# truongp-aws/neuronx-distributed-llama3_2

Measured on AMD Instinct MI355X. Metric: tokens/sec (whole node) Llama-3-8B TP=8 bf16 training at 1/2/4/8 MI355X, higher is better.
Workload: dtype bf16

## Files before the change

### neuronx_distributed_llama3_2_amd/csrc/dense_gemm.hip

```cpp
#include "gemm_tile.h"

#include <cstdlib>
#include <type_traits>

namespace nxd {
namespace dg {

constexpr int BM = 256, BN = 256, BK = 64, NT = 512;
constexpr int REG = 16384;
constexpr int BUF = 4 * REG;
constexpr int LDS_BYTES = 2 * BUF;
constexpr int R_ALO = 0, R_AHI = REG, R_BLO = 2 * REG, R_BHI = 3 * REG;

enum Layout { LNT = 0, LTN = 1 };
enum Epi { BF16 = 0, F32_ACC = 1, F32_ATOMIC = 2 };

struct Params {
  const uint16_t* a;
  const uint16_t* b;
  void* c;
  int M, N, K;
  int64_t lda, ldb, ldc;
  int mt, nt;
  int splits;
  int k_per_split;
  int band;
};

__device__ __forceinline__ int nt_swz(int r) { return (r >> 1) & 7; }

__device__ __forceinline__ bf16x8_t frag_nt(const char* reg, int r0, int s) {
  const int l = threadIdx.x & 63, r = r0 + (l & 15), ch = (l >> 4) + 4 * s;
  return __builtin_bit_cast(bf16x8_t, *reinterpret_cast<const u32x4_t*>(reg + r * 128 + ((ch ^ nt_swz(r)) << 4)));
}
template <int L>
__device__ __forceinline__ bf16x8_t frag(const char* reg, int x0, int s) {
  if constexpr (L == LNT) return frag_nt(reg, x0, s);
  else return frag_tr16<256>(reg, x0, 32 * s);
}

__device__ __forceinline__ void wait_regions(int younger) {
  switch (younger) {
    case 5: asm volatile("s_waitcnt vmcnt(10)" ::: "memory"); break;
    case 4: asm volatile("s_waitcnt vmcnt(8)" ::: "memory"); break;
    case 3: asm volatile("s_waitcnt vmcnt(6)" ::: "memory"); break;
    case 2: asm volatile("s_waitcnt vmcnt(4)" ::: "memory"); break;
    case 1: asm volatile("s_waitcnt vmcnt(2)" ::: "memory"); break;
    default: asm volatile("s_waitcnt vmcnt(0)" ::: "memory"); break;
  }
}

template <int L, int E>
__global__ void __launch_bounds__(NT, 1) gemm_kernel(Params p) {
  __shared__ __attribute__((aligned(16))) char smem[LDS_BYTES];
  const int tiles = p.mt * p.nt;
  const int id = xcd_remap(blockIdx.x, gridDim.x);
  const int split = id / tiles;
  int rt, ct;
  band_raster(id - split * tiles, p.mt, p.nt, p.band, rt, ct);
  const int m0 = rt * BM, n0 = ct * BN;
  const int k_begin = split * p.k_per_split;
  const int k_end = min(p.K, k_begin + p.k_per_split);
  const int nk = (k_end - k_begin) / BK;

  const int wid = threadIdx.x >> 6, lane = threadIdx.x & 63;
  const int wr = wid >> 2, wc = wid & 3;

  f32x4_t acc[4][4][2];
#pragma unroll
  for (int q = 0; q < 4; ++q)
#pragma unroll
    for (int i = 0; i < 4; ++i)
#pragma unroll
      for (int j = 0; j < 2; ++j) acc[q][i][j] = f32x4_t{0.f, 0.f, 0.f, 0.f};

  const uint16_t* sa[2][2];
  const uint16_t* sb[2][2];
#pragma unroll
  for (int h = 0; h < 2; ++h)
#pragma unroll
    for (int j = 0; j < 2; ++j) {
      const int piece = 2 * wid + j;
      if constexpr (L == LNT) {
        const int pr = 8 * piece + (lane >> 3), c = (lane & 7) ^ nt_swz(pr);
        sa[h][j] = p.a + (int64_t)min(m0 + 128 * h + pr, p.M - 1) * p.lda + k_begin + 8 * c;
        sb[h][j] = p.b + (int64_t)min(n0 + 128 * h + pr, p.N - 1) * p.ldb + k_begin + 8 * c;
      } else {
        const int pr = 4 * piece + (lane >> 4), c = (lane & 15) ^ tok_swz(pr);
        sa[h][j] = p.a + (int64_t)(k_begin + pr) * p.lda + min(m0 + 128 * h + 8 * c, p.M - 8);
        sb[h][j] = p.b + (int64_t)(k_begin + pr) * p.ldb + min(n0 + 128 * h + 8 * c, p.N - 8);
      }
    }
  const int64_t adv_a = L == LNT ? (int64_t)BK : (int64_t)BK * p.lda;
  const int64_t adv_b = L == LNT ? (int64_t)BK : (int64_t)BK * p.ldb;
  const uint32_t lds0 = lds_addr(smem);

  auto issue = [&](auto rc, int s) {
    constexpr int R = decltype(rc)::value;
    if (s >= nk) return;
    const uint32_t dst = lds0 + (s & 1) * BUF + (R == 0 ? R_ALO : R == 1 ? R_BLO : R == 2 ? R_BHI : R_AHI) + wid * 2048;
    if constexpr (R == 0 || R == 3) {
      constexpr int h = R == 0 ? 0 : 1;
      const int64_t o = (int64_t)s * adv_a;
      dma16(sa[h][0] + o, __builtin_amdgcn_readfirstlane(dst));
      dma16(sa[h][1] + o, __builtin_amdgcn_readfirstlane(dst + 1024));
    } else {
      constexpr int h = R == 1 ? 0 : 1;
      const int64_t o = (int64_t)s * adv_b;
      dma16(sb[h][0] + o, __builtin_amdgcn_readfirstlane(dst));
      dma16(sb[h][1] + o, __builtin_amdgcn_readfirstlane(dst + 1024));
    }
  };
  const int last = 4 * nk - 1;
  auto wait_for = [&](int need, int max_younger = 4) {
    if (need > last) return;
    wait_regions(min(max_younger, last - need));
  };

  using I0 = std::integral_constant<int, 0>;
  using I1 = std::integral_constant<int, 1>;
  using I2 = std::integral_constant<int, 2>;
  using I3 = std::integral_constant<int, 3>;
  bf16x8_t af[4][2], blo[2][2], bhi[2][2];

  issue(I0{}, 0); issue(I1{}, 0); issue(I2{}, 0); issue(I3{}, 0); issue(I0{}, 1); issue(I1{}, 1); issue(I2{}, 1);
  wait_for(1, 5);
  barrier();
#pragma unroll
  for (int i = 0; i < 4; ++i)
#pragma unroll
    for (int s = 0; s < 2; ++s) af[i][s] = frag<L>(smem + R_ALO, wr * 64 + 16 * i, s);
#pragma unroll
  for (int j = 0; j < 2; ++j)
#pragma unroll
    for (int s = 0; s < 2; ++s) blo[j][s] = frag<L>(smem + R_BLO, wc * 32 + 16 * j, s);
  wait_for(2);
  barrier();
  for (int t = 0; t < nk; ++t) {
    const char* buf = smem + (t & 1) * BUF;
    const char* nbuf = smem + ((t + 1) & 1) * BUF;
    issue(I3{}, t + 1);
#pragma unroll
    for (int s = 0; s < 2; ++s)
#pragma unroll
      for (int i = 0; i < 4; ++i) {
#pragma unroll
        for (int j = 0; j < 2; ++j)
          acc[0][i][j] = __builtin_amdgcn_mfma_f32_16x16x32_bf16(af[i][s], blo[j][s], acc[0][i][j], 0, 0, 0);
        if (i < 2) bhi[i][s] = frag<L>(buf + R_BHI, wc * 32 + 16 * i, s);
      }
    wait_for(4 * t + 3);
    barrier();
    issue(I0{}, t + 2);
#pragma unroll
    for (int s = 0; s < 2; ++s)
#pragma unroll
      for (int i = 0; i < 4; ++i) {
#pragma unroll
        for (int j = 0; j < 2; ++j)
          acc[1][i][j] = __builtin_amdgcn_mfma_f32_16x16x32_bf16(af[i][s], bhi[j][s], acc[1][i][j], 0, 0, 0);
        af[i][s] = frag<L>(buf + R_AHI, wr * 64 + 16 * i, s);
      }
    barrier();
    issue(I1{}, t + 2);
#pragma unroll
    for (int s = 0; s < 2; ++s)
#pragma unroll
      for (int i = 0; i < 4; ++i)
#pragma unroll
        for (int j = 0; j < 2; ++j)
          acc[2][i][j] = __builtin_amdgcn_mfma_f32_16x16x32_bf16(af[i][s], bhi[j][s], acc[2][i][j], 0, 0, 0);
    wait_for(4 * t + 5);
    barrier();
    issue(I2{}, t + 2);
#pragma unroll
    for (int s = 0; s < 2; ++s)
#pragma unroll
      for (int j = 0; j < 2; ++j) {
#pragma unroll
        for (int i = 0; i < 4; ++i) {
          acc[3][i][j] = __builtin_amdgcn_mfma_f32_16x16x32_bf16(af[i][s], blo[j][s], acc[3][i][j], 0, 0, 0);
          if (j == 1) af[i][s] = frag<L>(nbuf + R_ALO, wr * 64 + 16 * i, s);
        }
        blo[j][s] = frag<L>(nbuf + R_BLO, wc * 32 + 16 * j, s);
      }
    wait_for(4 * t + 6);
    barrier();
  }
  asm volatile("s_waitcnt vmcnt(0)" ::: "memory");
  __syncthreads();

  constexpr int LD = 36;
  float* slab = reinterpret_cast<float*>(smem) + wid * (64 * LD);
  const int crow = 4 * (lane >> 4), ccol = lane & 15;
#pragma unroll
  for (int qd = 0; qd < 4; ++qd) {
    const int rh = (qd == 2 || qd == 3) ? 1 : 0, ch = (qd == 1 || qd == 2) ? 1 : 0;
#pragma unroll
    for (int i = 0; i < 4; ++i)
#pragma unroll
      for (int j = 0; j < 2; ++j)
#pragma unroll
        for (int r = 0; r < 4; ++r) slab[(16 * i + crow + r) * LD + 16 * j + ccol] = acc[qd][i][j][r];
    __builtin_amdgcn_wave_barrier();
    const int row0 = m0 + 128 * rh + 64 * wr, col0 = n0 + 128 * ch + 32 * wc;
    if constexpr (E == F32_ATOMIC) {
      const int col = col0 + (lane & 31);
      float* cp = static_cast<float*>(p.c);
#pragma unroll 8
      for (int rr = 0; rr < 32; ++rr) {
        const int lr = 2 * rr + (lane >> 5), row = row0 + lr;
        const float v = slab[lr * LD + (lane & 31)];
        if (row < p.M && col < p.N) unsafeAtomicAdd(cp + (int64_t)row * p.ldc + col, v);
      }
    } else {
#pragma unroll
      for (int ps = 0; ps < 4; ++ps) {
        const int lr = 16 * ps + (lane >> 2), c8 = 8 * (lane & 3);
        const int row = row0 + lr, col = col0 + c8;
        const f32x4_t v0 = *reinterpret_cast<const f32x4_t*>(slab + lr * LD + c8);
        const f32x4_t v1 = *reinterpret_cast<const f32x4_t*>(slab + lr * LD + c8 + 4);
        if (row < p.M && col < p.N) {
          if constexpr (E == BF16) {
            u32x4_t o;
            o[0] = pack2bf(v0[0], v0[1]); o[1] = pack2bf(v0[2], v0[3]);
            o[2] = pack2bf(v1[0], v1[1]); o[3] = pack2bf(v1[2], v1[3]);
            *reinterpret_cast<u32x4_t*>(static_cast<uint16_t*>(p.c) + (int64_t)row * p.ldc + col) = o;
          } else {
            f32x4_t* cp = reinterpret_cast<f32x4_t*>(static_cast<float*>(p.c) + (int64_t)row * p.ldc + col);
            const f32x4_t c0 = cp[0], c1 = cp[1];
            cp[0] = c0 + v0;
            cp[1] = c1 + v1;
          }
        }
      }
    }
    __builtin_amdgcn_wave_barrier();
  }
}

static int env_int(const char* name, int dflt) {
  const char* e = getenv(name);
  return e ? atoi(e) : dflt;
}

}

int dense_gemm_choose_splits(int M, int N, int K) {
  const int tiles = ceil_div(M, dg::BM) * ceil_div(N, dg::BN);
  const int steps = K / dg::BK;
  const int64_t base = (int64_t)ceil_div(tiles, 256) * steps;
  int best = 1;
  int64_t best_cost = base;
  for (int s = 2; s <= 8 && s <= steps; ++s) {
    if (steps / s < 8) break;
    const int64_t cost = (int64_t)ceil_div(tiles * s, 256) * (ceil_div(steps, s) + 6);
    if (cost * 10 < best_cost * 9 && cost < best_cost) {
      best_cost = cost;
      best = s;
    }
  }
  return best;
}

int dense_gemm_launch(int layout, int epi, const void* a, int64_t lda, const void* b, int64_t ldb, void* c, int64_t ldc,
                      int M, int N, int K, int splits, hipStream_t stream) {
  if (M <= 0 || N <= 0 || K <= 0) return 0;
  if (K % dg::BK || N % 8 || lda % 8 || ldb % 8 || ldc % 4) return -1;
  if (layout == dg::LTN && M % 8) return -1;
  if (epi == dg::BF16 && ldc % 8) return -1;
  dg::Params p{};
  p.a = static_cast<const uint16_t*>(a);
  p.b = static_cast<const uint16_t*>(b);
  p.c = c;
  p.M = M; p.N = N; p.K = K;
  p.lda = lda; p.ldb = ldb; p.ldc = ldc;
  p.mt = ceil_div(M, dg::BM);
  p.nt = ceil_div(N, dg::BN);
  const int steps = K / dg::BK;
  if (epi != dg::F32_ATOMIC) splits = 1;
  else if (splits <= 0) splits = dense_gemm_choose_splits(M, N, K);
  splits = splits < 1 ? 1 : (splits > steps ? steps : splits);
  p.k_per_split = ceil_div(steps, splits) * dg::BK;
  p.splits = ceil_div(K, p.k_per_split);
  static const int band = [] { const int v = dg::env_int("NXD_DG_BAND", 8); return v > 0 ? v : 8; }();
  p.band = band;
  const int64_t nwg = (int64_t)p.mt * p.nt * p.splits;
  if (nwg > INT32_MAX) return -2;
#define NXD_DG_LAUNCH(LY, EP) \
  hipLaunchKernelGGL((dg::gemm_kernel<LY, EP>), dim3((unsigned)nwg), dim3(dg::NT), 0, stream, p)
  if (layout == dg::LNT) {
    if (epi == dg::BF16) NXD_DG_LAUNCH(dg::LNT, dg::BF16);
    else if (epi == dg::F32_ACC) NXD_DG_LAUNCH(dg::LNT, dg::F32_ACC);
    else NXD_DG_LAUNCH(dg::LNT, dg::F32_ATOMIC);
  } else {
    if (epi == dg::BF16) NXD_DG_LAUNCH(dg::LTN, dg::BF16);
    else if (epi == dg::F32_ACC) NXD_DG_LAUNCH(dg::LTN, dg::F32_ACC);
    else NXD_DG_LAUNCH(dg::LTN, dg::F32_ATOMIC);
  }
#undef NXD_DG_LAUNCH
  return hipGetLastError() == hipSuccess ? 0 : -3;
}

}
```

### neuronx_distributed_llama3_2_amd/ops/gemm.py

```python

from __future__ import annotations

import os

import torch

from ._ext import ext, use_native

_ENABLED = os.environ.get("NXD_TUNED_GEMM", "1") == "1"


def set_overlap_safe(enabled: bool) -> None:
    if not torch.cuda.is_available():
        return
    try:
        ext().gemm_set_no_streamk(1 if enabled else 0)
    except Exception:
        pass


def _native(*t: torch.Tensor) -> bool:
    return _ENABLED and use_native(*t) and all(x.dtype in (torch.bfloat16, torch.float16) for x in t)


def linear(x: torch.Tensor, w: torch.Tensor, bias=None, out: torch.Tensor = None) -> torch.Tensor:
    shape = x.shape[:-1] + (w.shape[0],)
    if _native(x, w) and x.stride(-1) == 1:
        x2 = x.reshape(-1, x.shape[-1])
        y = out if out is not None else torch.empty(shape, dtype=x.dtype, device=x.device)
        ext().gemm(x2, w.t(), y.view(-1, w.shape[0]), None, 1.0, 0.0)
        return y + bias if bias is not None else y
    y = torch.nn.functional.linear(x, w, bias)
    if out is not None:
        out.copy_(y)
        return out
    return y


def matmul(a: torch.Tensor, b: torch.Tensor, out: torch.Tensor = None) -> torch.Tensor:
    shape = a.shape[:-1] + (b.shape[1],)
    if _native(a, b) and a.stride(-1) == 1:
        a2 = a.reshape(-1, a.shape[-1])
        y = out if out is not None else torch.empty(shape, dtype=a.dtype, device=a.device)
        ext().gemm(a2, b, y.view(-1, b.shape[1]), None, 1.0, 0.0)
        return y
    y = torch.matmul(a, b)
    if out is not None:
        out.copy_(y)
        return out
    return y


_WGRAD_BF16 = os.environ.get("NXD_WGRAD_BF16", "0") == "1"
_scratch = {}


_WGRAD_T = os.environ.get("NXD_WGRAD_T", "1")


def _use_wgrad_t(go2: torch.Tensor, x2: torch.Tensor = None, K: int = None) -> bool:
    if _WGRAD_T == "0" or _WGRAD_BF16:
        return False
    T, N = go2.shape[0], go2.shape[1]
    K = x2.shape[1] if x2 is not None else K
    if T % 8 or N % 8 or K % 8 or go2.stride(-1) != 1 or go2.stride(0) % 8:
        return False
    if x2 is not None and (x2.stride(-1) != 1 or x2.stride(0) % 8):
        return False
    return _WGRAD_T == "2" or N * K / (N + K) > 1200


_WG_KERNEL = os.environ.get("NXD_WGRAD_KERNEL", "auto")
_WG_SKINNY = 1100.0
_WG_WIDE = 16000


def _use_wgrad_kernel(mg: torch.Tensor, go2: torch.Tensor, x2: torch.Tensor, has_copy: bool = False) -> bool:
    if _WG_KERNEL == "0" or x2 is None or not _native(go2, x2) or mg.dtype != torch.float32:
        return False
    T, M = go2.shape
    N = x2.shape[1]
    if T % 32 or M % 8 or N % 8 or go2.stride(1) != 1 or x2.stride(1) != 1 or mg.stride(1) != 1:
        return False
    if go2.stride(0) % 8 or x2.stride(0) % 8 or go2.data_ptr() % 16 or x2.data_ptr() % 16:
        return False
    return _WG_KERNEL == "1" or M * N / (M + N) < _WG_SKINNY or (not has_copy and max(M, N) >= _WG_WIDE)


_DENSE_WG = os.environ.get("NXD_DENSE_WGRAD", "auto")
_DENSE_WG_SKINNY = 2200.0


def _use_dense_wgrad(mg: torch.Tensor, go2: torch.Tensor, x2, has_copy: bool) -> bool:
    if _DENSE_WG == "0" or x2 is None or not _native(go2, x2) or mg.dtype != torch.float32:
        return False
    T, M = go2.shape
    N = x2.shape[1]
    if T % 64 or M % 8 or N % 8 or go2.stride(1) != 1 or x2.stride(1) != 1 or mg.stride(1) != 1:
        return False
    if go2.stride(0) % 8 or x2.stride(0) % 8 or mg.stride(0) % 4:
        return False
    if go2.data_ptr() % 16 or x2.data_ptr() % 16 or mg.data_ptr() % 16:
        return False
    return _DENSE_WG == "1" or (not has_copy and M * N / (M + N) < _DENSE_WG_SKINNY)


def _dense_wgrad(mg: torch.Tensor, go2: torch.Tensor, x2: torch.Tensor) -> None:
    C = ext()
    T, M = go2.shape
    splits = C.dense_gemm_splits(M, x2.shape[1], T)
    C.dense_gemm(1, 1 if splits == 1 else 2, go2, x2, mg, splits)


def _wgrad_scratch(n: int, dtype, device, tag: str = "") -> torch.Tensor:
    sid = torch.cuda.current_stream(device).stream_id if torch.device(device).type == "cuda" else 0
    key = (dtype, str(device), tag, sid)
    t = _scratch.get(key)
    if t is None or t.numel() < n:
        t = _scratch[key] = torch.empty(n, dtype=dtype, device=device)
    return t[:n]


def wgrad_accumulate_(mg: torch.Tensor, go2: torch.Tensor, x2, go_t: torch.Tensor = None,
                      x_t: torch.Tensor = None) -> None:
    has_copy = go_t is not None or x_t is not None
    if _use_dense_wgrad(mg, go2, x2, has_copy):
        _dense_wgrad(mg, go2, x2)
        return
    if _use_wgrad_kernel(mg, go2, x2, has_copy=has_copy):
        ext().wgrad_gemm(mg, go2, x2, 0)
        return
    if x_t is not None and not (x_t.dim() == 2 and x_t.is_contiguous() and x_t.shape[1] == go2.shape[0]):
        x_t = None
    if x2 is None and not (x_t is not None and _native(go2, x_t) and mg.is_contiguous()
                           and _use_wgrad_t(go2, K=x_t.shape[0])):
        x2 = x_t.t().contiguous()
        x_t = None
    if x2 is None or (_native(go2, x2) and mg.is_contiguous()):
        if x2 is None or _use_wgrad_t(go2, x2):
            T, N = go2.shape[0], go2.shape[1]
            K = x_t.shape[0] if x_t is not None else x2.shape[1]
            if go_t is not None and go_t.shape == (N, T) and go_t.is_contiguous() and go_t.dtype == go2.dtype:
                gt = go_t
            else:
                gt = transpose(go2, out=_wgrad_scratch(N * T, go2.dtype, go2.device, "gt").view(N, T))
            xt = x_t if x_t is not None else transpose(x2, out=_wgrad_scratch(K * T, x2.dtype, x2.device, "xt").view(K, T))
            ext().gemm(gt, xt.t(), mg, None, 1.0, 1.0)
            return
        if _WGRAD_BF16:
            tmp = _wgrad_scratch(mg.numel(), go2.dtype, go2.device).view(mg.shape)
            ext().gemm(go2.t(), x2, tmp, None, 1.0, 0.0)
            mg.add_(tmp)
            return
        ext().gemm(go2.t(), x2, mg, None, 1.0, 1.0)
        return
    if go2.is_cuda:
        torch.addmm(mg, go2.t(), x2, out_dtype=torch.float32, out=mg)
    else:
        mg.add_(go2.t().float().matmul(x2.float()))


_DGRAD_WT = os.environ.get("NXD_DGRAD_WT", "1") == "1"
_weight_epoch = [0]


def weights_updated() -> None:
    _weight_epoch[0] += 1


def transpose(src: torch.Tensor, out: torch.Tensor = None) -> torch.Tensor:
    dst = out if out is not None else torch.empty((src.shape[1], src.shape[0]), dtype=src.dtype, device=src.device)
    if use_native(src) and src.dtype == torch.bfloat16 and src.stride(-1) == 1 and src.shape[0] % 8 == 0 \
            and src.shape[1] % 8 == 0 and src.stride(0) % 8 == 0:
        ext().transpose_bf16(src, dst)
    else:
        dst.copy_(src.t())
    return dst


def _kmajor(weight: torch.Tensor) -> torch.Tensor:
    key = (_weight_epoch[0], weight._version, weight.data_ptr())
    wt = getattr(weight, "_nxd_wt", None)
    cur = torch.cuda.current_stream(weight.device)
    if wt is None or getattr(weight, "_nxd_wt_key", None) != key:
        if wt is None or wt.shape != (weight.shape[1], weight.shape[0]):
            wt = torch.empty((weight.shape[1], weight.shape[0]), dtype=weight.dtype, device=weight.device)
        transpose(weight.detach(), out=wt)
        weight._nxd_wt = wt
        weight._nxd_wt_key = key
        weight._nxd_wt_ev = torch.cuda.Event()
        weight._nxd_wt_ev.record(cur)
        weight._nxd_wt_stream = cur.stream_id
    elif getattr(weight, "_nxd_wt_stream", cur.stream_id) != cur.stream_id:
        cur.wait_event(weight._nxd_wt_ev)
        wt.record_stream(cur)
    return wt


def dgrad(go: torch.Tensor, weight: torch.Tensor, out: torch.Tensor = None) -> torch.Tensor:
    if _DGRAD_WT and _native(go, weight) and go.stride(-1) == 1 and weight.dim() == 2 and weight.shape[0] % 8 == 0 \
            and weight.shape[1] % 8 == 0 and weight.is_contiguous():
        wt = _kmajor(weight)
        return matmul(go, wt.t(), out=out)
    return matmul(go, weight, out=out)
```

Before: 21900.

## Restructure dense GEMM main loop with compile-time parity, SGPR-based DMA, and sched pins

Rewrites the dense GEMM kernel's K-loop into a compile-time unrolled two-tile pair with constant LDS offsets per buffer parity. Global-to-LDS loads now use a scalar base plus 32-bit per-lane offsets through inline asm setting m0. Fragment reads use precomputed LDS addresses with immediate offsets, and sched_group_barrier pins interleave MFMA with LDS reads. The aim is to cut address arithmetic and dynamic wait logic and to improve instruction interleaving. It adds a leading-dimension limit that falls back for large strides, plus optional setprio, at the cost of larger code and more register pressure.

```diff
diff --git a/neuronx_distributed_llama3_2_amd/csrc/dense_gemm.hip b/neuronx_distributed_llama3_2_amd/csrc/dense_gemm.hip
--- a/neuronx_distributed_llama3_2_amd/csrc/dense_gemm.hip
+++ b/neuronx_distributed_llama3_2_amd/csrc/dense_gemm.hip
@@ -3,14 +3,21 @@
 #include <cstdlib>
 #include <type_traits>
 
+#ifndef NXD_DG_SETPRIO
+#define NXD_DG_SETPRIO 0
+#endif
+#ifndef NXD_DG_SGB
+#define NXD_DG_SGB 1
+#endif
+
 namespace nxd {
 namespace dg {
 
 constexpr int BM = 256, BN = 256, BK = 64, NT = 512;
 constexpr int REG = 16384;
-constexpr int BUF = 4 * REG;
-constexpr int LDS_BYTES = 2 * BUF;
-constexpr int R_ALO = 0, R_AHI = REG, R_BLO = 2 * REG, R_BHI = 3 * REG;
+constexpr int LDS_BYTES = 8 * REG;
+constexpr int R_ALO = 0, R_AHI = 2 * REG, R_BLO = 4 * REG, R_BHI = 6 * REG;
+constexpr int64_t MAX_LD = (int64_t)1 << 22;
 
 enum Layout { LNT = 0, LTN = 1 };
 enum Epi { BF16 = 0, F32_ACC = 1, F32_ATOMIC = 2 };
@@ -29,25 +36,70 @@
 
 __device__ __forceinline__ int nt_swz(int r) { return (r >> 1) & 7; }
 
-__device__ __forceinline__ bf16x8_t frag_nt(const char* reg, int r0, int s) {
-  const int l = threadIdx.x & 63, r = r0 + (l & 15), ch = (l >> 4) + 4 * s;
-  return __builtin_bit_cast(bf16x8_t, *reinterpret_cast<const u32x4_t*>(reg + r * 128 + ((ch ^ nt_swz(r)) << 4)));
-}
+typedef __attribute__((address_space(3))) u32x4_t lds_u32x4_t;
+
+#pragma clang diagnostic push
+#pragma clang diagnostic ignored "-Winline-asm"
+template <int OFF>
+__device__ __forceinline__ void dma16s(uint32_t voff, const void* sbase, uint32_t sdst) {
+  asm volatile("s_add_u32 m0, %2, %3\n\ts_nop 0\n\tglobal_load_lds_dwordx4 %0, %1"
+               : : "v"(voff), "s"(sbase), "s"(sdst), "n"(OFF) : "memory", "m0", "scc");
+}
+#pragma clang diagnostic pop
+
+template <int L, int OFF>
+__device__ __forceinline__ bf16x8_t ld_frag(uint32_t base) {
+  if constexpr (L == LNT) {
+    return __builtin_bit_cast(bf16x8_t, *reinterpret_cast<const lds_u32x4_t*>((uintptr_t)(base + OFF)));
+  } else {
+    const short4_t lo = __builtin_amdgcn_ds_read_tr16_b64_v4i16(reinterpret_cast<lds_short4_t*>((uintptr_t)(base + OFF)));
+    const short4_t hi = __builtin_amdgcn_ds_read_tr16_b64_v4i16(reinterpret_cast<lds_short4_t*>((uintptr_t)(base + OFF + 4 * 256)));
+    const short __attribute__((ext_vector_type(8))) a8 = {lo[0], lo[1], lo[2], lo[3], hi[0], hi[1], hi[2], hi[3]};
+    return __builtin_bit_cast(bf16x8_t, a8);
+  }
+}
+
 template <int L>
-__device__ __forceinline__ bf16x8_t frag(const char* reg, int x0, int s) {
-  if constexpr (L == LNT) return frag_nt(reg, x0, s);
-  else return frag_tr16<256>(reg, x0, 32 * s);
-}
-
-__device__ __forceinline__ void wait_regions(int younger) {
-  switch (younger) {
-    case 5: asm volatile("s_waitcnt vmcnt(10)" ::: "memory"); break;
-    case 4: asm volatile("s_waitcnt vmcnt(8)" ::: "memory"); break;
-    case 3: asm volatile("s_waitcnt vmcnt(6)" ::: "memory"); break;
-    case 2: asm volatile("s_waitcnt vmcnt(4)" ::: "memory"); break;
-    case 1: asm volatile("s_waitcnt vmcnt(2)" ::: "memory"); break;
-    default: asm volatile("s_waitcnt vmcnt(0)" ::: "memory"); break;
-  }
+__device__ __forceinline__ uint32_t frag_base(int x0, int v) {
+  const int l = threadIdx.x & 63;
+  if constexpr (L == LNT) {
+    const int r = x0 + (l & 15), ch = (l >> 4) + 4 * v;
+    return r * 128 + ((ch ^ nt_swz(r)) << 4);
+  } else {
+    const int g = l >> 4, i = l & 15, q = i >> 2, pp = i & 3;
+    const int col = x0 + 4 * pp, t = 8 * g + q;
+    return t * 256 + 16 * ((col >> 3) ^ tok_swz(t)) + 8 * (pp & 1);
+  }
+}
+
+template <int V> using IC = std::integral_constant<int, V>;
+
+template <int N>
+__device__ __forceinline__ void wait_vm() {
+  if constexpr (N == 8) asm volatile("s_waitcnt vmcnt(8)" ::: "memory");
+  else if constexpr (N == 10) asm volatile("s_waitcnt vmcnt(10)" ::: "memory");
+  else if constexpr (N == 4) asm volatile("s_waitcnt vmcnt(4)" ::: "memory");
+  else if constexpr (N == 2) asm volatile("s_waitcnt vmcnt(2)" ::: "memory");
+  else asm volatile("s_waitcnt vmcnt(0)" ::: "memory");
+}
+
+__device__ __forceinline__ void burst_begin() {
+#if NXD_DG_SETPRIO
+  __builtin_amdgcn_s_setprio(1);
+#endif
+}
+__device__ __forceinline__ void burst_end() {
+#if NXD_DG_SETPRIO
+  __builtin_amdgcn_s_setprio(0);
+#endif
+}
+
+template <int L, int nm, int nf>
+__device__ __forceinline__ void pin() {
+#if NXD_DG_SGB
+  if constexpr (nm > 0) __builtin_amdgcn_sched_group_barrier(0x008, nm, 0);
+  if constexpr (nf > 0) __builtin_amdgcn_sched_group_barrier(0x100, nf * (L == LNT ? 1 : 2), 0);
+#endif
 }
 
 template <int L, int E>
@@ -74,8 +126,16 @@
 #pragma unroll
       for (int j = 0; j < 2; ++j) acc[q][i][j] = f32x4_t{0.f, 0.f, 0.f, 0.f};
 
-  const uint16_t* sa[2][2];
-  const uint16_t* sb[2][2];
+  const uint16_t* abase;
+  const uint16_t* bbase;
+  uint32_t oa[2][2], ob[2][2];
+  if constexpr (L == LNT) {
+    abase = p.a + (int64_t)m0 * p.lda + k_begin;
+    bbase = p.b + (int64_t)n0 * p.ldb + k_begin;
+  } else {
+    abase = p.a + (int64_t)k_begin * p.lda + m0;
+    bbase = p.b + (int64_t)k_begin * p.ldb + n0;
+  }
 #pragma unroll
   for (int h = 0; h < 2; ++h)
 #pragma unroll
@@ -83,86 +143,101 @@
       const int piece = 2 * wid + j;
       if constexpr (L == LNT) {
         const int pr = 8 * piece + (lane >> 3), c = (lane & 7) ^ nt_swz(pr);
-        sa[h][j] = p.a + (int64_t)min(m0 + 128 * h + pr, p.M - 1) * p.lda + k_begin + 8 * c;
-        sb[h][j] = p.b + (int64_t)min(n0 + 128 * h + pr, p.N - 1) * p.ldb + k_begin + 8 * c;
+        oa[h][j] = 2u * ((uint32_t)(min(m0 + 128 * h + pr, p.M - 1) - m0) * (uint32_t)p.lda + 8 * c);
+        ob[h][j] = 2u * ((uint32_t)(min(n0 + 128 * h + pr, p.N - 1) - n0) * (uint32_t)p.ldb + 8 * c);
       } else {
         const int pr = 4 * piece + (lane >> 4), c = (lane & 15) ^ tok_swz(pr);
-        sa[h][j] = p.a + (int64_t)(k_begin + pr) * p.lda + min(m0 + 128 * h + 8 * c, p.M - 8);
-        sb[h][j] = p.b + (int64_t)(k_begin + pr) * p.ldb + min(n0 + 128 * h + 8 * c, p.N - 8);
+        oa[h][j] = 2u * ((uint32_t)pr * (uint32_t)p.lda + (uint32_t)(min(m0 + 128 * h + 8 * c, p.M - 8) - m0));
+        ob[h][j] = 2u * ((uint32_t)pr * (uint32_t)p.ldb + (uint32_t)(min(n0 + 128 * h + 8 * c, p.N - 8) - n0));
       }
     }
   const int64_t adv_a = L == LNT ? (int64_t)BK : (int64_t)BK * p.lda;
   const int64_t adv_b = L == LNT ? (int64_t)BK : (int64_t)BK * p.ldb;
   const uint32_t lds0 = lds_addr(smem);
-
-  auto issue = [&](auto rc, int s) {
-    constexpr int R = decltype(rc)::value;
-    if (s >= nk) return;
-    const uint32_t dst = lds0 + (s & 1) * BUF + (R == 0 ? R_ALO : R == 1 ? R_BLO : R == 2 ? R_BHI : R_AHI) + wid * 2048;
+  const uint32_t sdst = __builtin_amdgcn_readfirstlane(lds0 + wid * 2048);
+
+  auto issue = [&](auto rc, auto parc) __attribute__((always_inline)) {
+    constexpr int R = decltype(rc)::value, PAR = decltype(parc)::value;
+    constexpr int off = PAR * REG + (R == 0 ? R_ALO : R == 1 ? R_BLO : R == 2 ? R_BHI : R_AHI);
     if constexpr (R == 0 || R == 3) {
       constexpr int h = R == 0 ? 0 : 1;
-      const int64_t o = (int64_t)s * adv_a;
-      dma16(sa[h][0] + o, __builtin_amdgcn_readfirstlane(dst));
-      dma16(sa[h][1] + o, __builtin_amdgcn_readfirstlane(dst + 1024));
+      dma16s<off>(oa[h][0], abase, sdst);
+      dma16s<off + 1024>(oa[h][1], abase, sdst);
     } else {
       constexpr int h = R == 1 ? 0 : 1;
-      const int64_t o = (int64_t)s * adv_b;
-      dma16(sb[h][0] + o, __builtin_amdgcn_readfirstlane(dst));
-      dma16(sb[h][1] + o, __builtin_amdgcn_readfirstlane(dst + 1024));
-    }
-  };
-  const int last = 4 * nk - 1;
-  auto wait_for = [&](int need, int max_younger = 4) {
-    if (need > last) return;
-    wait_regions(min(max_younger, last - need));
-  };
-
-  using I0 = std::integral_constant<int, 0>;
-  using I1 = std::integral_constant<int, 1>;
-  using I2 = std::integral_constant<int, 2>;
-  using I3 = std::integral_constant<int, 3>;
+      dma16s<off>(ob[h][0], bbase, sdst);
+      dma16s<off + 1024>(ob[h][1], bbase, sdst);
+    }
+  };
+
+  constexpr int NA = L == LNT ? 2 : 4;
+  uint32_t fa[NA], fb[2];
+#pragma unroll
+  for (int v = 0; v < NA; ++v) {
+    fa[v] = lds0 + frag_base<L>(wr * 64 + (L == LNT ? 0 : 16 * v), v);
+    asm volatile("" : "+v"(fa[v]));
+  }
+#pragma unroll
+  for (int v = 0; v < 2; ++v) {
+    fb[v] = lds0 + R_BLO + frag_base<L>(wc * 32 + (L == LNT ? 0 : 16 * v), v);
+    asm volatile("" : "+v"(fb[v]));
+  }
+  auto lda_frag = [&](auto parc, auto roc, auto ic, auto sc) __attribute__((always_inline)) {
+    constexpr int O = decltype(parc)::value * REG + decltype(roc)::value, i = decltype(ic)::value, s = decltype(sc)::value;
+    if constexpr (L == LNT) return ld_frag<L, O + 2048 * i>(fa[s]);
+    else return ld_frag<L, O + 8192 * s>(fa[i]);
+  };
+  auto ldb_frag = [&](auto parc, auto roc, auto jc, auto sc) __attribute__((always_inline)) {
+    constexpr int O = decltype(parc)::value * REG + decltype(roc)::value - R_BLO, j = decltype(jc)::value, s = decltype(sc)::value;
+    if constexpr (L == LNT) return ld_frag<L, O + 2048 * j>(fb[s]);
+    else return ld_frag<L, O + 8192 * s>(fb[j]);
+  };
+
   bf16x8_t af[4][2], blo[2][2], bhi[2][2];
 
-  issue(I0{}, 0); issue(I1{}, 0); issue(I2{}, 0); issue(I3{}, 0); issue(I0{}, 1); issue(I1{}, 1); issue(I2{}, 1);
-  wait_for(1, 5);
-  barrier();
-#pragma unroll
-  for (int i = 0; i < 4; ++i)
-#pragma unroll
-    for (int s = 0; s < 2; ++s) af[i][s] = frag<L>(smem + R_ALO, wr * 64 + 16 * i, s);
-#pragma unroll
-  for (int j = 0; j < 2; ++j)
-#pragma unroll
-    for (int s = 0; s < 2; ++s) blo[j][s] = frag<L>(smem + R_BLO, wc * 32 + 16 * j, s);
-  wait_for(2);
-  barrier();
-  for (int t = 0; t < nk; ++t) {
-    const char* buf = smem + (t & 1) * BUF;
-    const char* nbuf = smem + ((t + 1) & 1) * BUF;
-    issue(I3{}, t + 1);
-#pragma unroll
-    for (int s = 0; s < 2; ++s)
-#pragma unroll
-      for (int i = 0; i < 4; ++i) {
+  auto for_s = [&](auto f) __attribute__((always_inline)) { f(IC<0>{}); f(IC<1>{}); };
+  auto for_i = [&](auto f) __attribute__((always_inline)) { f(IC<0>{}); f(IC<1>{}); f(IC<2>{}); f(IC<3>{}); };
+
+  auto tile = [&](auto parc, auto dc) __attribute__((always_inline)) {
+    constexpr int PAR = decltype(parc)::value, D = decltype(dc)::value;
+    using P = IC<PAR>;
+    using Q = IC<PAR ^ 1>;
+    if constexpr (D >= 1) {
+      issue(IC<3>{}, Q{});
+      abase += adv_a;
+    }
+    burst_begin();
+    for_s([&](auto sc) __attribute__((always_inline)) {
+      for_i([&](auto ic) __attribute__((always_inline)) {
+        constexpr int s = decltype(sc)::value, i = decltype(ic)::value;
 #pragma unroll
         for (int j = 0; j < 2; ++j)
           acc[0][i][j] = __builtin_amdgcn_mfma_f32_16x16x32_bf16(af[i][s], blo[j][s], acc[0][i][j], 0, 0, 0);
-        if (i < 2) bhi[i][s] = frag<L>(buf + R_BHI, wc * 32 + 16 * i, s);
-      }
-    wait_for(4 * t + 3);
-    barrier();
-    issue(I0{}, t + 2);
-#pragma unroll
-    for (int s = 0; s < 2; ++s)
-#pragma unroll
-      for (int i = 0; i < 4; ++i) {
+        if constexpr (i < 2) bhi[i][s] = ldb_frag(P{}, IC<R_BHI>{}, ic, sc);
+      });
+    });
+#pragma unroll
+    for (int s = 0; s < 2; ++s) { pin<L, 2, 1>(); pin<L, 2, 1>(); pin<L, 4, 0>(); }
+    burst_end();
+    wait_vm<D >= 1 ? 8 : 0>();
+    barrier();
+    if constexpr (D >= 2) issue(IC<0>{}, P{});
+    burst_begin();
+    for_s([&](auto sc) __attribute__((always_inline)) {
+      for_i([&](auto ic) __attribute__((always_inline)) {
+        constexpr int s = decltype(sc)::value, i = decltype(ic)::value;
 #pragma unroll
         for (int j = 0; j < 2; ++j)
           acc[1][i][j] = __builtin_amdgcn_mfma_f32_16x16x32_bf16(af[i][s], bhi[j][s], acc[1][i][j], 0, 0, 0);
-        af[i][s] = frag<L>(buf + R_AHI, wr * 64 + 16 * i, s);
-      }
-    barrier();
-    issue(I1{}, t + 2);
+        af[i][s] = lda_frag(P{}, IC<R_AHI>{}, ic, sc);
+      });
+    });
+#pragma unroll
+    for (int k = 0; k < 8; ++k) pin<L, 2, 1>();
+    burst_end();
+    barrier();
+    if constexpr (D >= 2) issue(IC<1>{}, P{});
+    burst_begin();
 #pragma unroll
     for (int s = 0; s < 2; ++s)
 #pragma unroll
@@ -170,23 +245,78 @@
 #pragma unroll
         for (int j = 0; j < 2; ++j)
           acc[2][i][j] = __builtin_amdgcn_mfma_f32_16x16x32_bf16(af[i][s], bhi[j][s], acc[2][i][j], 0, 0, 0);
-    wait_for(4 * t + 5);
-    barrier();
-    issue(I2{}, t + 2);
-#pragma unroll
-    for (int s = 0; s < 2; ++s)
-#pragma unroll
-      for (int j = 0; j < 2; ++j) {
-#pragma unroll
-        for (int i = 0; i < 4; ++i) {
+    burst_end();
+    if constexpr (D >= 1) wait_vm<D >= 2 ? 8 : 4>();
+    barrier();
+    if constexpr (D >= 2) {
+      issue(IC<2>{}, P{});
+      bbase += adv_b;
+    }
+    burst_begin();
+    for_s([&](auto sc) __attribute__((always_inline)) {
+      for_s([&](auto jc) __attribute__((always_inline)) {
+        for_i([&](auto ic) __attribute__((always_inline)) {
+          constexpr int s = decltype(sc)::value, j = decltype(jc)::value, i = decltype(ic)::value;
           acc[3][i][j] = __builtin_amdgcn_mfma_f32_16x16x32_bf16(af[i][s], blo[j][s], acc[3][i][j], 0, 0, 0);
-          if (j == 1) af[i][s] = frag<L>(nbuf + R_ALO, wr * 64 + 16 * i, s);
-        }
-        blo[j][s] = frag<L>(nbuf + R_BLO, wc * 32 + 16 * j, s);
-      }
-    wait_for(4 * t + 6);
-    barrier();
-  }
+          if constexpr (j == 1 && D >= 1) af[i][s] = lda_frag(Q{}, IC<R_ALO>{}, ic, sc);
+        });
+        if constexpr (D >= 1) blo[decltype(jc)::value][decltype(sc)::value] = ldb_frag(Q{}, IC<R_BLO>{}, jc, sc);
+      });
+    });
+    if constexpr (D >= 1) {
+#pragma unroll
+      for (int s = 0; s < 2; ++s) { pin<L, 4, 1>(); pin<L, 1, 1>(); pin<L, 1, 1>(); pin<L, 1, 1>(); pin<L, 1, 2>(); }
+    }
+    burst_end();
+    if constexpr (D >= 1) wait_vm<D >= 2 ? 8 : 2>();
+    barrier();
+  };
+
+  auto first_frags = [&](auto parc) __attribute__((always_inline)) {
+    for_s([&](auto sc) __attribute__((always_inline)) {
+      for_i([&](auto ic) __attribute__((always_inline)) {
+        af[decltype(ic)::value][decltype(sc)::value] = lda_frag(parc, IC<R_ALO>{}, ic, sc);
+      });
+      for_s([&](auto jc) __attribute__((always_inline)) {
+        blo[decltype(jc)::value][decltype(sc)::value] = ldb_frag(parc, IC<R_BLO>{}, jc, sc);
+      });
+    });
+  };
+  auto prologue = [&](auto parc) __attribute__((always_inline)) {
+    using P = decltype(parc);
+    using Q = IC<P::value ^ 1>;
+    issue(IC<0>{}, P{}); issue(IC<1>{}, P{}); issue(IC<2>{}, P{}); issue(IC<3>{}, P{});
+    abase += adv_a;
+    bbase += adv_b;
+    issue(IC<0>{}, Q{}); issue(IC<1>{}, Q{}); issue(IC<2>{}, Q{});
+    bbase += adv_b;
+    wait_vm<10>();
+    barrier();
+    first_frags(P{});
+    wait_vm<8>();
+    barrier();
+  };
+  if (nk == 1) {
+    issue(IC<0>{}, IC<1>{}); issue(IC<1>{}, IC<1>{}); issue(IC<2>{}, IC<1>{}); issue(IC<3>{}, IC<1>{});
+    wait_vm<4>();
+    barrier();
+    first_frags(IC<1>{});
+    wait_vm<2>();
+    barrier();
+  } else {
+    if (nk & 1) {
+      prologue(IC<1>{});
+      tile(IC<1>{}, IC<2>{});
+    } else {
+      prologue(IC<0>{});
+    }
+    for (int it = (nk - 2) >> 1; it > 0; --it) {
+      tile(IC<0>{}, IC<2>{});
+      tile(IC<1>{}, IC<2>{});
+    }
+    tile(IC<0>{}, IC<1>{});
+  }
+  tile(IC<1>{}, IC<0>{});
   asm volatile("s_waitcnt vmcnt(0)" ::: "memory");
   __syncthreads();
 
@@ -269,6 +399,7 @@
   if (K % dg::BK || N % 8 || lda % 8 || ldb % 8 || ldc % 4) return -1;
   if (layout == dg::LTN && M % 8) return -1;
   if (epi == dg::BF16 && ldc % 8) return -1;
+  if (lda >= dg::MAX_LD || ldb >= dg::MAX_LD) return -1;
   dg::Params p{};
   p.a = static_cast<const uint16_t*>(a);
   p.b = static_cast<const uint16_t*>(b);
diff --git a/neuronx_distributed_llama3_2_amd/ops/gemm.py b/neuronx_distributed_llama3_2_amd/ops/gemm.py
--- a/neuronx_distributed_llama3_2_amd/ops/gemm.py
+++ b/neuronx_distributed_llama3_2_amd/ops/gemm.py
@@ -91,6 +91,12 @@
 _DENSE_WG_SKINNY = 2200.0
 
 
+def _dense_wgrad_rule(T: int, M: int, N: int, has_copy: bool) -> bool:
+    if _DENSE_WG == "1":
+        return True
+    return not has_copy and M * N / (M + N) < _DENSE_WG_SKINNY
+
+
 def _use_dense_wgrad(mg: torch.Tensor, go2: torch.Tensor, x2, has_copy: bool) -> bool:
     if _DENSE_WG == "0" or x2 is None or not _native(go2, x2) or mg.dtype != torch.float32:
         return False
@@ -102,7 +108,7 @@
         return False
     if go2.data_ptr() % 16 or x2.data_ptr() % 16 or mg.data_ptr() % 16:
         return False
-    return _DENSE_WG == "1" or (not has_copy and M * N / (M + N) < _DENSE_WG_SKINNY)
+    return _dense_wgrad_rule(T, M, N, has_copy)
 
 
 def _dense_wgrad(mg: torch.Tensor, go2: torch.Tensor, x2: torch.Tensor) -> None:
```

Result: slower. 21100 (-3.6%).
